# vrettasm/VGPA

Measured on AMD Instinct MI355X. Metric: fwd+bwd sweeps/sec (free-energy+grad eval), Lorenz96 D=40 N=1000, higher is better.
Workload: dtype f64; 1 GPU; Lorenz96 D=40, RK4, Np=1001 (BASELINE configs[2]); batch_per_gpu=512, kernels=mfma

## Files before the change

### vgpa_amd/csrc/energy.hip

```cpp
#include "vgpa_internal.h"
#include "energy_small.h"
#include "chol_wave.h"

namespace vgpa {
namespace {

constexpr int NT = 256;

__global__ void __launch_bounds__(NT) k_energy_1d(EnergyArgs a) {
  const int t = blockIdx.x * NT + threadIdx.x;
  const int prob = blockIdx.y;
  if (t >= a.Np) return;
  const size_t o = (size_t)prob * a.Np + t;
  const double la = a.A[(size_t)prob * a.strideA + t], ob = a.b[(size_t)prob * a.strideB + t], m = a.m[o], s = a.S[o];
  Energy1d r;
  const double th = a.theta_v ? a.theta_v[(size_t)prob * kMaxTheta] : a.theta[0];
  const double sg = a.sigma1_v ? a.sigma1_v[prob] : a.sigma1;
  if (a.model == VGPA_MODEL_OU) energy_1d<VGPA_MODEL_OU>(th, sg, la, ob, m, s, r);
  else energy_1d<VGPA_MODEL_DW>(th, sg, la, ob, m, s, r);
  if (a.hyp_only) { a.hyp[o] = r.hyp; return; }
  a.e_t[o] = r.e_t;
  a.Ef[o] = r.ef;
  if (a.Edf) a.Edf[o] = r.edf;
  a.dEm[o] = r.dm;
  a.dEs[o] = r.ds;
  if (a.hyp) a.hyp[o] = r.hyp;
}

__global__ void __launch_bounds__(64) k_energy_l63(EnergyArgs a) {
  const int t = blockIdx.x * 64 + threadIdx.x;
  const int prob = blockIdx.y;
  if (t >= a.Np) return;
  const size_t o = (size_t)prob * a.Np + t;
  const double* At = a.A + (size_t)prob * a.strideA + (size_t)t * 9;
  const double* bt = a.b + (size_t)prob * a.strideB + (size_t)t * 3;
  const double* mt = a.m + o * 3;
  const double* St = a.S + o * 9;
  double Av[9], bv[3], mv[3], Sv[9], isg[3];
  const double* th = a.theta_v ? a.theta_v + (size_t)prob * kMaxTheta : a.theta;
  const double* isgp = a.isg + (size_t)prob * a.isg_stride;
#pragma unroll
  for (int e = 0; e < 9; e++) { Av[e] = At[e]; Sv[e] = St[e]; }
#pragma unroll
  for (int i = 0; i < 3; i++) { bv[i] = bt[i]; mv[i] = mt[i]; isg[i] = isgp[i]; }
  EnergyL63 r;
  if (a.hyp) energy_l63<true>(th, isg, Av, bv, mv, Sv, r); else energy_l63<false>(th, isg, Av, bv, mv, Sv, r);
  if (a.hyp_only) {
    double* hp = a.hyp + o * 6;
#pragma unroll
    for (int i = 0; i < 6; i++) hp[i] = r.hyp[i];
    return;
  }
  a.e_t[o] = r.e_t;
  double* dm = a.dEm + o * 3;
  dm[0] = r.dm[0]; dm[1] = r.dm[1]; dm[2] = r.dm[2];
  double* ds = a.dEs + o * 9;
  ds[0] = r.ds[0]; ds[1] = r.ds[1]; ds[2] = r.ds[2];
  ds[3] = r.ds[1]; ds[4] = r.ds[3]; ds[5] = r.ds[4];
  ds[6] = r.ds[2]; ds[7] = r.ds[4]; ds[8] = r.ds[5];
  double* ef = a.Ef + o * 3;
// ... 73 lines not shown
      if (!any) continue;
      const double af = pa[kk * 4 * LD + 4 * I];
#pragma unroll
      for (int q = 0; q < g::NQ; q++)
        if (kk >= 4 * q && !(TRI == 1 && 4 * q + 3 < I) && !(TRI == 2 && 4 * q > I)) acc[q * NB + I] = __builtin_amdgcn_mfma_f64_4x4x4f64(af, bq[q], acc[q * NB + I], 0, 0, 0);
    }
    if (g::NLEFT > 0 && kk >= 4 * g::NQ) {
#pragma unroll
      for (int v = 0; v < g::NLEFT; v++) {
        if (MODE == 1 && kk < v * g::G) continue;
        if (TRI == 2 && v * g::G + g::G - 1 < 4 * g::NQ) continue;
        int ib = v * g::G + ileft;
        ib = ib < NB ? ib : NB - 1;
        const double af = pa[kk * 4 * LD + 4 * ib];
        acc[NB * g::NQ + v] = __builtin_amdgcn_mfma_f64_4x4x4f64(af, bl, acc[NB * g::NQ + v], 0, 0, 0);
      }
    }
  }
}

template <int NB>
__device__ __forceinline__ void wave_gemm_elem(int u, int& row, int& col, bool& ok) {
  using g = WaveGemmGeo<NB>;
  const int l = threadIdx.x & 63, r4 = l >> 4, c4 = l & 3, b = (l >> 2) & 3;
  constexpr int rem = g::REM ? g::REM : 1;
  int Ib, Jb;
  if (u < NB * g::NQ) {
    const int q = u / NB;
    Ib = u - q * NB; Jb = 4 * q + b; ok = true;
  } else {
    const int v = u - NB * g::NQ;
    Ib = v * g::G + b / rem; Jb = 4 * g::NQ + b % rem;
    ok = (b < g::G * g::REM) && (Ib < NB);
  }
  row = 4 * Ib + r4; col = 4 * Jb + c4;
}

struct L96Lds {
  double *Lm, *Gm, *mv, *bv, *am, *sg, *vv, *dl, *qq, *rd;
};

__host__ __device__ inline int l96_dp(int D) { return 4 * ((D + 3) / 4); }
__host__ __device__ inline int l96_ld(int D) { return l96_dp(D) + 1; }
__host__ __device__ inline size_t l96_lds_doubles(int D) {
  return (size_t)2 * l96_dp(D) * l96_ld(D) + 7 * (size_t)l96_dp(D) + (2 * D + 1) + 8 + 4 * (size_t)l96_dp(D);
}

template <int NB>
__global__ void __launch_bounds__(64) k_energy_l96(EnergyArgs a) {
  extern __shared__ __attribute__((aligned(16))) double smem[];
  const int D = a.D, M = 2 * D + 1;
  constexpr int Dp = 4 * NB, LD = Dp + 1;
  const int l = threadIdx.x;
  const long long wid = blockIdx.x;
  const int prob = (int)(wid / a.Np), t = (int)(wid - (long long)prob * a.Np);
  const size_t o = (size_t)prob * a.Np + t;
  L96Lds S;
  S.Lm = smem; S.Gm = S.Lm + Dp * LD; S.mv = S.Gm + Dp * LD; S.bv = S.mv + Dp; S.am = S.bv + Dp; S.sg = S.am + Dp;
  S.dl = S.sg + Dp; S.qq = S.dl + Dp; S.rd = S.qq + Dp; S.vv = S.rd + Dp;
  const double* At = a.A + (size_t)prob * a.strideA + (size_t)t * D * D;
  const double* St = a.S + o * D * D;
  const double theta = a.theta_v ? lds_const(a.theta_v, prob * kMaxTheta) : a.theta[0];
  const double kappa = 1.05 * D, c = D + kappa;
  const bool act = l < D;
  const bool pad = l < Dp;
  const int li = pad ? l : Dp - 1;

  for (int e = l; e < Dp * LD; e += 64) { S.Lm[e] = 0.0; S.Gm[e] = 0.0; }
  if (pad) { S.mv[l] = 0.0; S.bv[l] = 0.0; S.sg[l] = 0.0; S.am[l] = 0.0; S.dl[l] = 0.0; S.qq[l] = 0.0; S.rd[l] = 1.0; }
  wave_sync();
  {
    constexpr int EPL = (Dp * Dp + 63) / 64;
    const int DD = D * D;
    const unsigned magic = ((1u << 20) + (unsigned)D - 1u) / (unsigned)D;
#pragma unroll
    for (int q0 = 0; q0 < EPL; q0 += 9) {
      double sv[9], av[9];
#pragma unroll
      for (int u = 0; u < 9; u++) {
        const int e = l + 64 * (q0 + u);
        const bool in = (q0 + u < EPL) && (e < DD);
        sv[u] = in ? St[e] : 0.0;
        av[u] = in ? At[e] : 0.0;
      }
#pragma unroll
      for (int u = 0; u < 9; u++) {
        const int e = l + 64 * (q0 + u);
        if ((q0 + u < EPL) && (e < DD)) {
          const int r = (int)(((unsigned)e * magic) >> 20), cc = e - r * D;
          S.Lm[r * LD + cc] = c * sv[u];
          S.Gm[cc * LD + r] = av[u];
        }
      }
    }
  }
  if (l >= D && pad) S.Lm[l * LD + l] = 1.0;
  if (act) { S.mv[l] = a.m[o * D + l]; S.bv[l] = a.b[(size_t)prob * a.strideB + (size_t)t * D + l]; S.sg[l] = a.isg[(size_t)prob * a.isg_stride + l]; }
  wave_sync();

  const int r4 = l >> 4, c4 = l & 3, b = (l >> 2) & 3;
  bool bad = false;
  double myrd = 1.0;
  const double* lrow_b = S.Lm + (4 * b + c4) * LD + r4;
  double* lout_b = S.Lm + (4 * b + r4) * LD + c4;
#pragma unroll
  for (int p = 0; p < NB; p++) {
    const int j0 = 4 * p;
    if (p > 0) {
      const double* brow = S.Lm + (j0 + c4) * LD + r4;
#pragma unroll
      for (int u = 0; p + 4 * u < NB; u++) {
        const bool full = p + 4 * u + 3 < NB;
        const bool rowok = full || (p + 4 * u + b < NB);
        const double* arow = full ? lrow_b + 4 * (p + 4 * u) * LD
                                  : S.Lm + (4 * (rowok ? p + 4 * u + b : NB - 1) + c4) * LD + r4;
        double uacc = 0.0;
#pragma unroll
        for (int kk = 0; kk < p; kk++) uacc = __builtin_amdgcn_mfma_f64_4x4x4f64(arow[4 * kk], brow[4 * kk], uacc, 0, 0, 0);
        if (rowok) lout_b[4 * (p + 4 * u) * LD + j0] -= uacc;
      }
      wave_sync();
    }
    chol_panel_pivots<LD>(S.Lm, myrd, j0, l, li, pad);
    wave_sync();
  }
  if (pad) S.rd[l] = myrd;
  wave_sync();
// ... 103 lines not shown
  if (l == 0) a.e_t[o] = e_t;
  wave_sync();

  const double* l4_a = S.Lm + c4 * LD + r4;
  const double* xd_a = xdiag + 4 * c4 + r4;
  const double* xd_d = xdiag + 4 * r4 + c4;
#pragma unroll
  for (int I = 0; I < NB; I++) {
    const double* arow = l4_a + 4 * I * LD;
    const double xd = xd_a[16 * I];
    const double xdd = xd_d[16 * I];
#pragma unroll
    for (int u = 0; 4 * u < NB; u++) {
      const int Jb = 4 * u + b;
      const bool colok = (4 * u + 3 < NB) || (Jb < NB);
      double* xcol = S.Gm + r4 * LD + 4 * (colok ? Jb : NB - 1) + c4;
      double xo = 0.0;
      if (4 * u <= I) {
        double tacc = 0.0;
#pragma unroll
        for (int K = 4 * u; K < I; K++) tacc = __builtin_amdgcn_mfma_f64_4x4x4f64(arow[4 * K], xcol[4 * K * LD], tacc, 0, 0, 0);
        const double prod = __builtin_amdgcn_mfma_f64_4x4x4f64(xd, tacc, 0.0, 0, 0, 0);
        xo = (Jb < I) ? -prod : ((Jb == I) ? xdd : 0.0);
      }
      if (colok) xcol[4 * I * LD] = xo;
    }
    wave_sync();
  }

  {
    double s = 0.0;
    for (int k = 0; k < Dp; k++) s = __builtin_fma(S.Gm[k * LD + li], S.dl[k], s);
    if (act) a.dEm[o * D + l] = 0.5 * c * s;
  }
  double* ds = a.dEs + o * D * D;
  {
    double acc[WaveGemmGeo<NB>::NU];
    wave_gemm<NB, 1>(S.Gm, S.Gm, LD, acc, S.qq);
#pragma unroll
    for (int u = 0; u < WaveGemmGeo<NB>::NU; u++) {
      int row, col; bool ok;
      wave_gemm_elem<NB>(u, row, col, ok);
      if (ok && row < D && col < D && (row <= col || !a.ds_upper)) ds[row * D + col] = 0.5 * c * acc[u];
    }
  }

  if (act) {
    const int i = l, ip1 = wrap(i + 1, D), im1 = wrap(i - 1, D), im2 = wrap(i - 2, D);
    const double cxx = St[ip1 * D + im1] - St[im2 * D + im1];
    a.Ef[o * D + i] = cxx + (S.mv[ip1] - S.mv[im2]) * S.mv[im1] - S.mv[i] + theta;
  }
  if (a.Edf) {
    double* ed = a.Edf + o * D * D;
    for (int e = l; e < D * D; e += 64) {
      const int k = e / D, j = e - k * D;
      const int kp1 = wrap(k + 1, D), km1 = wrap(k - 1, D), km2 = wrap(k - 2, D);
      double v = 0.0;
      if (j == k) v = -1.0;
      if (j == kp1) v = S.mv[km1];
      if (j == km2) v = -S.mv[km1];
      if (j == km1) v = S.mv[kp1] - S.mv[km2];
      ed[e] = v;
    }
  }
}

__host__ __device__ inline bool l96r_compact(int D) { return (D + 3) / 4 == 10; }
__host__ __device__ inline size_t l96r_lds_doubles(int D) {
  const size_t dp = l96_dp(D);
  if (l96r_compact(D)) return dp * l96_ld(D) + 5 * dp;
  return dp * l96_ld(D) + 6 * dp + 9 * dp;
}
template <int R>
__device__ __forceinline__ double row_ror_blocks(double v) {
  typedef int i2_t __attribute__((ext_vector_type(2)));
  i2_t x = __builtin_bit_cast(i2_t, v), y;
  y[0] = __builtin_amdgcn_mov_dpp(x[0], 0x120 + 4 * R, 0xf, 0xf, false);
  y[1] = __builtin_amdgcn_mov_dpp(x[1], 0x120 + 4 * R, 0xf, 0xf, false);
  return __builtin_bit_cast(double, y);
}

struct TriRowTab { unsigned char r[2080]; };
constexpr TriRowTab make_tri_row_tab() {
  TriRowTab t{};
  int e = 0;
  for (int r = 0; r < 64; r++)
    for (int c = 0; c <= r; c++) t.r[e++] = (unsigned char)r;
  return t;
}
__device__ __constant__ TriRowTab kTriRow = make_tri_row_tab();

template <int NB, bool TG = false>
__global__ void __launch_bounds__(64) __attribute__((amdgpu_waves_per_eu(NB <= 10 ? 3 : 2, NB <= 10 ? 3 : 2))) k_energy_l96_r(EnergyArgs a) {
  extern __shared__ __attribute__((aligned(16))) double smem[];
  const int D = a.D, M = 2 * D + 1;
  constexpr int Dp = 4 * NB, LD = Dp + 1, NUU = (NB + 3) / 4;
  const int l = threadIdx.x;
  const long long wid = blockIdx.x;
  const int prob = (int)(wid / a.Np);
  const int t = (int)(wid - (long long)prob * a.Np);
  const size_t o = (size_t)prob * a.Np + t;
  L96Lds S;
  constexpr bool CMP = (NB == 10);
  S.Lm = smem; S.Gm = nullptr; S.mv = S.Lm + Dp * LD; S.bv = S.mv + Dp; S.am = S.bv + Dp; S.sg = nullptr;
  S.dl = S.am + Dp; S.qq = S.dl + Dp; S.rd = CMP ? nullptr : S.qq + Dp; S.vv = CMP ? nullptr : S.rd + Dp;
  double* pv = S.vv;
  double* pw = CMP ? nullptr : pv + 4 * Dp;
  double* gb2 = CMP ? nullptr : pw + 4 * Dp;
  double* xdiag = pv;
  auto cg2 = [&](int j) -> double* { return S.Lm + j * LD + Dp; };
  auto cps = [&](int minus, int j) -> double* { return S.Lm + (4 + 2 * minus + (j >= 20 ? 1 : 0)) * LD + (j >= 20 ? j : 20 + j); };
  auto cxd = [&](int I, int r, int c) -> double* { return S.Lm + ((I < 6 ? 0 : 4) + r) * LD + 4 * (I < 6 ? I + 4 : I - 1) + c; };
  const double* At = a.A + (size_t)prob * a.strideA + (size_t)t * D * D;
  const bool spk = a.s_packed != 0;
  const int PK = tri_off(D);
  const double* St = a.S + o * (spk ? PK : D * D);
  const double theta = a.theta_v ? lds_const(a.theta_v, prob * kMaxTheta) : a.theta[0];
  const double kappa = 1.05 * D, c = D + kappa;
  const bool act = l < D;
  const bool pad = l < Dp;
  const int li = pad ? l : Dp - 1;
  const int r4 = l >> 4, c4 = l & 3, b = (l >> 2) & 3;

  constexpr int NUE = 0;
  double af[NUU][NB];
  const int klim = (D - r4 + 3) >> 2;
  auto load_af = [&](int u) {
    const int row = 16 * u + (l & 15);
    const double* ap = At + row * D + r4;
    const int kl = row < D ? klim : 0;
#pragma unroll
    for (int K = 0; K < NB; K++) af[u][K] = (K < kl) ? ap[4 * K] : 0.0;
  };

  double sxa = 0.0, sxb = 0.0, v_m = 0.0, v_b = 0.0, v_sg = 0.0;
  double nsxa = 0.0, nsxb = 0.0;
  const int f_ip1 = wrap(l + 1, D), f_im1 = wrap(l - 1, D), f_im2 = wrap(l - 2, D);
  if (act) v_sg = a.isg[(size_t)prob * a.isg_stride + l];
  auto load_vectors = [&]() {
    if (act) {
      sxa = St[f_ip1 * D + f_im1];
      sxb = St[f_im2 * D + f_im1];
      v_m = a.m[o * D + l];
      v_b = a.b[(size_t)prob * a.strideB + (size_t)t * D + l];
    }
  };
  constexpr int EPK = (Dp * (Dp + 1) / 2 + 63) / 64;
  double sv[EPK];
  int rr[EPK];
  auto request = [&](int tn) {
    const size_t on = (size_t)prob * a.Np + tn;
    const double* Sn = a.S + on * PK;
#pragma unroll
    for (int q = 0; q < EPK; q++) {
      const int e = l + 64 * q;
      sv[q] = e < PK ? Sn[e] : 0.0;
      rr[q] = kTriRow.r[e < PK ? e : 0];
    }
    if (act) {
      nsxa = Sn[tri_idx(f_ip1, f_im1)];
      nsxb = Sn[tri_idx(f_im2, f_im1)];
      v_m = a.m[on * D + l];
      v_b = a.b[(size_t)prob * a.strideB + (size_t)tn * D + l];
    }
  };
  if (spk) request(t);

  if (spk) {
    if (D != Dp) {
      for (int e = l; e < Dp * LD; e += 64) S.Lm[e] = 0.0;
      wave_sync();
    }
    sxa = nsxa; sxb = nsxb;
#pragma unroll
    for (int q = 0; q < EPK; q++) {
      const int e = l + 64 * q;
      if (e < PK) {
        const int r = rr[q];
        S.Lm[r * LD + (e - tri_off(r))] = c * sv[q];
      }
    }
  } else if (D == Dp) {
    constexpr int RCH = Dp <= 44 ? Dp : 32;
    const double* sp = St + li;
#pragma unroll
    for (int q0 = 0; q0 < Dp; q0 += RCH) {
      double sv[RCH];
#pragma unroll
      for (int u = 0; u < RCH; u++) sv[u] = (q0 + u < Dp) ? sp[(q0 + u) * Dp] : 0.0;
      if (q0 == 0) load_vectors();
      if (pad) {
#pragma unroll
        for (int u = 0; u < RCH; u++)
          if (q0 + u < Dp) S.Lm[(q0 + u) * LD + l] = c * sv[u];
      }
    }
  } else {
    load_vectors();
    for (int e = l; e < Dp * LD; e += 64) S.Lm[e] = 0.0;
    wave_sync();
    constexpr int EPL = (Dp * Dp + 63) / 64;
    constexpr int CH = (NB <= 11) ? EPL : 13;
    const int DD = D * D;
    const unsigned magic = ((1u << 20) + (unsigned)D - 1u) / (unsigned)D;
#pragma unroll
    for (int q0 = 0; q0 < EPL; q0 += CH) {
      double sv[CH];
#pragma unroll
      for (int u = 0; u < CH; u++) {
        const int e = l + 64 * (q0 + u);
        const bool in = (q0 + u < EPL) && (e < DD);
        sv[u] = in ? St[e] : 0.0;
      }
#pragma unroll
      for (int u = 0; u < CH; u++) {
        const int e = l + 64 * (q0 + u);
        if ((q0 + u < EPL) && (e < DD)) {
          const int r = (int)(((unsigned)e * magic) >> 20), cc = e - r * D;
          S.Lm[r * LD + cc] = c * sv[u];
        }
      }
    }
  }
  if (l >= D && pad) S.Lm[l * LD + l] = 1.0;
  if (pad) { S.mv[l] = v_m; S.bv[l] = v_b; S.am[l] = 0.0; }
  wave_sync();

  bool bad = false;
  double myrd = 1.0;
  const double* lrow_b = S.Lm + (4 * b + c4) * LD + r4;
  double* lout_b = S.Lm + (4 * b + r4) * LD + c4;
#pragma unroll
  for (int p = 0; p < NB; p++) {
    const int j0 = 4 * p;
    if (p > 0) {
      const double* brow = S.Lm + (j0 + c4) * LD + r4;
#pragma unroll
      for (int u = 0; p + 4 * u < NB; u++) {
        const bool full = p + 4 * u + 3 < NB;
        const bool rowok = full || (p + 4 * u + b < NB);
        const double* arow = full ? lrow_b + 4 * (p + 4 * u) * LD
                                  : S.Lm + (4 * (rowok ? p + 4 * u + b : NB - 1) + c4) * LD + r4;
        double uacc = 0.0;
#pragma unroll
        for (int kk = 0; kk < p; kk++) uacc = __builtin_amdgcn_mfma_f64_4x4x4f64(arow[4 * kk], brow[4 * kk], uacc, 0, 0, 0);
        if (rowok) lout_b[4 * (p + 4 * u) * LD + j0] -= uacc;
      }
      wave_sync();
    }
    chol_panel_pivots<LD>(S.Lm, myrd, j0, l, li, pad);
    wave_sync();
  }
  if (!CMP && pad) S.rd[l] = myrd;
  wave_sync();
  bad = __any(!(myrd > 0.0 && myrd < __builtin_inf()));
  if (bad) {
    if (l == 0) atomicOr(a.status + prob, 1);
    return;
  }
#pragma unroll
  for (int u = NUE; u < NUU; u++) load_af(u);

  double amr[NUU], gacc[NUU][NB];
#pragma unroll
  for (int u = 0; u < NUU; u++) {
    amr[u] = 0.0;
#pragma unroll
    for (int J = 0; J < NB; J++) gacc[u][J] = 0.0;
  }
#pragma unroll
  for (int pass = 0; pass < (NUE < NUU ? 2 : 1); pass++) {
    const int u0 = pass == 0 ? 0 : NUE, u1 = pass == 0 ? NUE : NUU;
#pragma unroll
    for (int K = 0; K < NB; K++) {
      const double mk = S.mv[4 * K + r4];
#pragma unroll
      for (int u = u0; u < u1; u++) amr[u] = __builtin_amdgcn_mfma_f64_4x4x4f64(af[u][K], mk, amr[u], 0, 0, 0);
      const double* lk = S.Lm + (4 * K + r4) * LD + c4;
#pragma unroll
      for (int J = 0; J <= K; J++) {
        const double lf = lk[4 * J];
#pragma unroll
        for (int u = u0; u < u1; u++) gacc[u][J] = __builtin_amdgcn_mfma_f64_4x4x4f64(af[u][K], lf, gacc[u][J], 0, 0, 0);
      }
    }
  }
#pragma unroll
  for (int u = 0; u < NUU; u++) {
    const int i = 16 * u + 4 * b + r4;
    if (c4 == 0 && i < D) { S.am[i] = amr[u]; if (!TG && a.Am) a.Am[o * D + i] = amr[u]; }
  }
  if constexpr (TG) wave_sync();

  if constexpr (!TG) {
#pragma unroll
  for (int u = 0; u < NUU; u++) {
    if (u == 0 || (16 * u <= Dp - 1 && 16 * u + 15 >= Dp - 4)) {
      const int i = 16 * u + 4 * b + r4;
      if constexpr (CMP) {
        if (i == D - 1) {
#pragma unroll
          for (int J = 0; J < NB; J++) *cg2(4 * J + c4) = gacc[u][J];
        }
      }
      double* gdst = (i == 0) ? S.dl : ((i == 1) ? S.qq : ((i == D - 1 && !CMP) ? gb2 : nullptr));
      if (gdst) {
#pragma unroll
        for (int J = 0; J < NB; J++) gdst[4 * J + c4] = gacc[u][J];
      }
    }
  }
  }
  double tg_edge = 0.0;
  if constexpr (TG) {
    const double w0 = kappa / c, w1 = 1.0 / (2.0 * c);
    auto col_of = [&](int q) { return q == 0 ? 0 : (q <= D ? q - 1 : q - 1 - D); };
    auto sgn_of = [&](int q) { return q == 0 ? 0.0 : (q <= D ? 1.0 : -1.0); };
    auto chi = [&](int q, int i) { return S.mv[i] + sgn_of(q) * S.Lm[i * LD + col_of(q)]; };
    const int jc = act ? l : 0;
    const int pP = 1 + jc, pM = 1 + D + jc;
    const int pPm = pP - 1, pPp = pP + 1;
    const int pMm = pM - 1, pMp = wrap(pM + 1, M);
    const double P0 = chi(pPm, D - 2), P1 = chi(pPm, D - 1), P2 = chi(pP, 0), P3 = chi(pP, 1), P4 = chi(pP, 2);
    const double N0 = chi(pMm, D - 2), N1 = chi(pMm, D - 1), N2 = chi(pM, 0), N3 = chi(pM, 1), N4 = chi(pM, 2);
    const double Q0 = chi(pP, D - 3), Q1 = chi(pP, D - 2), Q2 = chi(pP, D - 1), Q3 = chi(pPp, 0);
    const double R0 = chi(pM, D - 3), R1 = chi(pM, D - 2), R2 = chi(pM, D - 1), R3 = chi(pMp, 0);
    double bsum = 0.0;
    {
      const double lin = S.am[0] - S.bv[0];
      bsum += lane_value(v_sg, 0) * ((((P3 - P0) * P1 - P2 + theta) + lin) + (((N3 - N0) * N1 - N2 + theta) + lin));
    }
    {
      const double lin = S.am[1] - S.bv[1];
      bsum += lane_value(v_sg, 1) * ((((P4 - P1) * P2 - P3 + theta) + lin) + (((N4 - N1) * N2 - N3 + theta) + lin));
    }
    {
      const double lin = S.am[D - 1] - S.bv[D - 1];
      bsum += lane_value(v_sg, D - 1) * ((((Q3 - Q0) * Q1 - Q2 + theta) + lin) + (((R3 - R0) * R1 - R2 + theta) + lin));
    }
    double part = 0.0;
    if (act) {
      const int i = l;
      const double xm2 = (i >= 2) ? S.mv[i - 2] : chi(M - 1, D - 2 + i);
      const double xm1 = (i >= 1) ? S.mv[i - 1] : chi(M - 1, D - 1);
      const double x1 = (i + 1 < D) ? S.mv[i + 1] : chi(1, 0);
      const double r0 = ((x1 - xm2) * xm1 - S.mv[i] + theta) + S.am[i] - S.bv[i];
      part += w1 * bsum + w0 * (v_sg * r0);
    }
    tg_edge = part;
  }
  double vp[NB], vm[NB];
  double tgi = 0.0;
#pragma unroll
  for (int J = 0; J < NB; J++) { vp[J] = 0.0; vm[J] = 0.0; }
  {
#pragma clang fp contract(fast)
#pragma unroll
  for (int u = 0; u < NUU; u++) {
    const int i = 16 * u + 4 * b + r4;
    const bool ok = (i >= 2) && (i <= D - 2);
    const int ir = ok ? i : 2;
    const double mm2 = S.mv[ir - 2], mm1 = S.mv[ir - 1], m0 = S.mv[ir], m1 = S.mv[ir + 1];
    const double sgr = __shfl(v_sg, ir, 64);
    const double bvi = S.bv[ir], sgi = ok ? sgr : 0.0, ami = amr[u];
    const double dm = m1 - mm2;
    const double base = dm * mm1 - m0 + theta + ami - bvi;
    const double* lp = S.Lm + (ir - 2) * LD + c4;
#pragma unroll
    for (int J = 0; J < NB; J++) {
      const double e2 = lp[4 * J], e1 = lp[LD + 4 * J], e0 = lp[2 * LD + 4 * J], ep = lp[3 * LD + 4 * J];
      const double gi = gacc[u][J];
      const double dl = ep - e2;
      const double ev = base + dl * e1;
      const double od = dm * e1 + (dl * mm1 + (gi - e0));
      vp[J] = vp[J] + sgi * (ev * ev + od * od);
      vm[J] = vm[J] + sgi * (ev * od);
      if constexpr (TG) tgi = tgi + ((4 * J + c4 < D) ? sgi : 0.0) * ev;
      if (J == NB / 2 - 1 || J == NB - 1) __builtin_amdgcn_sched_barrier(0);
    }
  }
  }
  if constexpr (TG) {
    const double part = wave_sum(tg_edge + 2.0 * (1.0 / (2.0 * c)) * tgi);
    if (l == 0) a.tg[o] = part;
    return;
  }
  {
    double rp[NB], rm[NB];
#pragma unroll
    for (int J = 0; J < NB; J++) {
      rp[J] = __builtin_amdgcn_mfma_f64_4x4x4f64(1.0, vp[J], 0.0, 0, 0, 0);
      rm[J] = __builtin_amdgcn_mfma_f64_4x4x4f64(1.0, vm[J], 0.0, 0, 0, 0);
    }
    if constexpr (CMP) {
#pragma unroll
      for (int J = 0; J < NB; J++) {
        const double p1 = rp[J] + row_ror_blocks<1>(rp[J]), m1 = rm[J] + row_ror_blocks<1>(rm[J]);
        rp[J] = p1 + row_ror_blocks<2>(p1);
        rm[J] = m1 + row_ror_blocks<2>(m1);
      }
      wave_sync();
      if (r4 == 0 && b == 0) {
#pragma unroll
        for (int J = 0; J < NB; J++) {
          *cps(0, 4 * J + c4) = rp[J];
          *cps(1, 4 * J + c4) = rm[J];
        }
      }
    } else
    if (r4 == 0) {
#pragma unroll
      for (int J = 0; J < NB; J++) {
        pv[b * Dp + 4 * J + c4] = rp[J];
        pw[b * Dp + 4 * J + c4] = rm[J];
      }
    }
  }
  wave_sync();

  double vplus = 0.0, vminus = 0.0, v0 = 0.0;
  {
    auto col_of = [&](int q) { return q == 0 ? 0 : (q <= D ? q - 1 : q - 1 - D); };
    auto sgn_of = [&](int q) { return q == 0 ? 0.0 : (q <= D ? 1.0 : -1.0); };
    auto chi = [&](int q, int i) { return S.mv[i] + sgn_of(q) * S.Lm[i * LD + col_of(q)]; };
    const int jc = act ? l : 0;
    {
      double s1, s2;
      if constexpr (CMP) { s1 = *cps(0, jc); s2 = *cps(1, jc); }
      else {
        s1 = (pv[jc] + pv[Dp + jc]) + (pv[2 * Dp + jc] + pv[3 * Dp + jc]);
        s2 = (pw[jc] + pw[Dp + jc]) + (pw[2 * Dp + jc] + pw[3 * Dp + jc]);
      }
      vplus = s1 + 2.0 * s2;
      vminus = s1 - 2.0 * s2;
    }
    const int pP = 1 + jc, pM = 1 + D + jc;
    const int pPm = pP - 1, pPp = pP + 1;
    const int pMm = pM - 1, pMp = wrap(pM + 1, M);
    {
      const double P0 = chi(pPm, D - 2), P1 = chi(pPm, D - 1), P2 = chi(pP, 0), P3 = chi(pP, 1), P4 = chi(pP, 2);
      const double N0 = chi(pMm, D - 2), N1 = chi(pMm, D - 1), N2 = chi(pM, 0), N3 = chi(pM, 1), N4 = chi(pM, 2);
      const double Q0 = chi(pP, D - 3), Q1 = chi(pP, D - 2), Q2 = chi(pP, D - 1), Q3 = chi(pPp, 0);
      const double R0 = chi(pM, D - 3), R1 = chi(pM, D - 2), R2 = chi(pM, D - 1), R3 = chi(pMp, 0);
      const double g0 = S.dl[jc], g1 = S.qq[jc], g2 = CMP ? *cg2(jc) : gb2[jc];
      {
        const double ami = S.am[0], bvi = S.bv[0], sgi = lane_value(v_sg, 0);
        const double ra = ((P3 - P0) * P1 - P2 + theta) + (ami + g0) - bvi;
        const double rb = ((N3 - N0) * N1 - N2 + theta) + (ami - g0) - bvi;
        vplus = __builtin_fma(sgi, ra * ra, vplus);
        vminus = __builtin_fma(sgi, rb * rb, vminus);
      }
      {
        const double ami = S.am[1], bvi = S.bv[1], sgi = lane_value(v_sg, 1);
        const double ra = ((P4 - P1) * P2 - P3 + theta) + (ami + g1) - bvi;
        const double rb = ((N4 - N1) * N2 - N3 + theta) + (ami - g1) - bvi;
        vplus = __builtin_fma(sgi, ra * ra, vplus);
        vminus = __builtin_fma(sgi, rb * rb, vminus);
      }
      {
        const double ami = S.am[D - 1], bvi = S.bv[D - 1], sgi = lane_value(v_sg, D - 1);
        const double ra = ((Q3 - Q0) * Q1 - Q2 + theta) + (ami + g2) - bvi;
        const double rb = ((R3 - R0) * R1 - R2 + theta) + (ami - g2) - bvi;
        vplus = __builtin_fma(sgi, ra * ra, vplus);
        vminus = __builtin_fma(sgi, rb * rb, vminus);
      }
    }
    if (act) {
      const int i = l;
      const double xm2 = (i >= 2) ? S.mv[i - 2] : chi(M - 1, D - 2 + i);
      const double xm1 = (i >= 1) ? S.mv[i - 1] : chi(M - 1, D - 1);
      const double x1 = (i + 1 < D) ? S.mv[i + 1] : chi(1, 0);
      const double r0 = ((x1 - xm2) * xm1 - S.mv[i] + theta) + S.am[i] - S.bv[i];
      v0 = v_sg * (r0 * r0);
    }
    v0 = wave_sum(v0);
  }
  const double w0 = kappa / c, w1 = 1.0 / (2.0 * c);
  const double e_part = act ? (vplus + vminus) : 0.0;
  const double e_t = 0.5 * (w0 * v0 + w1 * wave_sum(e_part));
  wave_sync();
  if (pad) {
    S.dl[l] = act ? w1 * (vplus - vminus) : 0.0;
    S.qq[l] = act ? 0.5 * c * (w1 * (vplus + vminus)) - e_t : 0.0;
  }
  if (l == 0) a.e_t[o] = e_t;
  const int l4 = l < NB ? 4 * l : 0;
  const double rd0 = CMP ? __shfl(myrd, l4, 64) : 0.0, rd1 = CMP ? __shfl(myrd, l4 + 1, 64) : 0.0;
  const double rd2 = CMP ? __shfl(myrd, l4 + 2, 64) : 0.0, rd3 = CMP ? __shfl(myrd, l4 + 3, 64) : 0.0;
  if (l < NB) {
    const double* tb = S.Lm + (4 * l) * LD + 4 * l;
    const double x00 = CMP ? rd0 : S.rd[4 * l], x11 = CMP ? rd1 : S.rd[4 * l + 1], x22 = CMP ? rd2 : S.rd[4 * l + 2], x33 = CMP ? rd3 : S.rd[4 * l + 3];
    const double t10 = tb[LD], t20 = tb[2 * LD], t21 = tb[2 * LD + 1], t30 = tb[3 * LD], t31 = tb[3 * LD + 1], t32 = tb[3 * LD + 2];
    const double x10 = -(t10 * x00) * x11;
    const double x21 = -(t21 * x11) * x22;
    const double x32 = -(t32 * x22) * x33;
    const double x20 = -(t20 * x00 + t21 * x10) * x22;
    const double x31 = -(t31 * x11 + t32 * x21) * x33;
    const double x30 = -(t30 * x00 + t31 * x10 + t32 * x20) * x33;
    if constexpr (CMP) {
      double* x0 = cxd(l, 0, 0);
      x0[0] = x00; x0[1] = 0.0; x0[2] = 0.0; x0[3] = 0.0;
      x0[LD] = x10; x0[LD + 1] = x11; x0[LD + 2] = 0.0; x0[LD + 3] = 0.0;
      x0[2 * LD] = x20; x0[2 * LD + 1] = x21; x0[2 * LD + 2] = x22; x0[2 * LD + 3] = 0.0;
      x0[3 * LD] = x30; x0[3 * LD + 1] = x31; x0[3 * LD + 2] = x32; x0[3 * LD + 3] = x33;
    } else {
    double* xo = xdiag + 16 * l;
    xo[0] = x00; xo[1] = 0.0; xo[2] = 0.0; xo[3] = 0.0;
    xo[4] = x10; xo[5] = x11; xo[6] = 0.0; xo[7] = 0.0;
    xo[8] = x20; xo[9] = x21; xo[10] = x22; xo[11] = 0.0;
    xo[12] = x30; xo[13] = x31; xo[14] = x32; xo[15] = x33;
    }
  }
  wave_sync();

  const double* l4_a = S.Lm + c4 * LD + r4;
  const double* xd_a = xdiag + 4 * c4 + r4;
  const double* xd_d = xdiag + 4 * r4 + c4;
#pragma unroll
  for (int I = 0; I < NB; I++) {
    const double* arow = l4_a + 4 * I * LD;
    const double xd = CMP ? *cxd(I, c4, r4) : xd_a[16 * I];
    const double xdd = CMP ? *cxd(I, r4, c4) : xd_d[16 * I];
    double xo[NUU];
#pragma unroll
    for (int u = 0; u < NUU; u++) {
      const int Jb = 4 * u + b;
      const bool colok = (4 * u + 3 < NB) || (Jb < NB);
      const double* xcol = S.Lm + r4 * LD + 4 * (colok ? Jb : NB - 1) + c4;
      xo[u] = 0.0;
      if (4 * u <= I) {
        double tacc = 0.0;
#pragma unroll
        for (int K = 4 * u; K < I; K++) tacc = __builtin_amdgcn_mfma_f64_4x4x4f64(arow[4 * K], xcol[4 * K * LD], tacc, 0, 0, 0);
        const double prod = __builtin_amdgcn_mfma_f64_4x4x4f64(xd, tacc, 0.0, 0, 0, 0);
        xo[u] = (Jb < I) ? -prod : ((Jb == I) ? xdd : 0.0);
      }
    }
#pragma unroll
    for (int u = 0; u < NUU; u++) {
      const int Jb = 4 * u + b;
      const bool colok = (4 * u + 3 < NB) || (Jb < NB);
      if (colok && (!CMP || Jb <= I)) S.Lm[(4 * I + r4) * LD + 4 * Jb + c4] = xo[u];
    }
    wave_sync();
  }

  {
    double s = 0.0;
    if constexpr (CMP) {
      const bool z0 = li < 4, z1 = li < 8;
#pragma unroll
      for (int k = 0; k < 8; k++) s = __builtin_fma((k < 4 ? z0 : z1) ? S.Lm[k * LD + li] : 0.0, S.dl[k], s);
      for (int k = 8; k < Dp; k++) s = __builtin_fma(S.Lm[k * LD + li], S.dl[k], s);
    } else
    for (int k = 0; k < Dp; k++) s = __builtin_fma(S.Lm[k * LD + li], S.dl[k], s);
    if (act) a.dEm[o * D + l] = 0.5 * c * s;
  }
  double* ds = a.dEs + o * D * D;
  {
    double acc[WaveGemmGeo<NB>::NU];
    if (a.ds_packed) {
      using gg = WaveGemmGeo<NB>;
      double* dsp = a.dEs + o * PK;
      wave_gemm<NB, 1, 2>(S.Lm, S.Lm, LD, acc, S.qq);
#pragma unroll
      for (int u = 0; u < gg::NU; u++) {
        if (u < NB * gg::NQ && 4 * (u / NB) > u % NB) continue;
        if (u >= NB * gg::NQ && (u - NB * gg::NQ) * gg::G + gg::G - 1 < 4 * gg::NQ) continue;
        int row, col; bool ok;
        wave_gemm_elem<NB>(u, row, col, ok);
        if (ok && row < D && col <= row) dsp[tri_off(row) + col] = 0.5 * c * acc[u];
      }
    } else if (a.ds_upper) {
      wave_gemm<NB, 1, 1>(S.Lm, S.Lm, LD, acc, S.qq);
#pragma unroll
      for (int u = 0; u < WaveGemmGeo<NB>::NU; u++) {
        if (u < NB * WaveGemmGeo<NB>::NQ && 4 * (u / NB) + 3 < u % NB) continue;
        int row, col; bool ok;
        wave_gemm_elem<NB>(u, row, col, ok);
        if (ok && row < D && col < D && row <= col) ds[row * D + col] = 0.5 * c * acc[u];
      }
    } else {
      wave_gemm<NB, 1>(S.Lm, S.Lm, LD, acc, S.qq);
#pragma unroll
      for (int u = 0; u < WaveGemmGeo<NB>::NU; u++) {
        int row, col; bool ok;
        wave_gemm_elem<NB>(u, row, col, ok);
        if (ok && row < D && col < D) ds[row * D + col] = 0.5 * c * acc[u];
      }
    }
  }

  if (act) {
    const int i = l, ip1 = wrap(i + 1, D), im1 = wrap(i - 1, D), im2 = wrap(i - 2, D);
    const double cxx = sxa - sxb;
    a.Ef[o * D + i] = cxx + (S.mv[ip1] - S.mv[im2]) * S.mv[im1] - S.mv[i] + theta;
  }
  if (a.Edf) {
    double* ed = a.Edf + o * D * D;
    for (int e = l; e < D * D; e += 64) {
      const int k = e / D, j = e - k * D;
      const int kp1 = wrap(k + 1, D), km1 = wrap(k - 1, D), km2 = wrap(k - 2, D);
      double v = 0.0;
      if (j == k) v = -1.0;
      if (j == kp1) v = S.mv[km1];
      if (j == km2) v = -S.mv[km1];
      if (j == km1) v = S.mv[kp1] - S.mv[km2];
      ed[e] = v;
    }
  }
}

__global__ void __launch_bounds__(NT) k_edf_dense(EnergyArgs a) {
  const int D = a.D;
  const int t = blockIdx.x, prob = blockIdx.y;
  const size_t o = (size_t)prob * a.Np + t;
  const double* mv = a.m + o * D;
  double* ed = a.Edf + o * D * D;
  const double* th = a.theta_v ? a.theta_v + (size_t)prob * kMaxTheta : a.theta;
  for (int e = threadIdx.x; e < D * D; e += NT) {
    const int k = e / D, j = e - k * D;
    double v = 0.0;
    if (a.model == VGPA_MODEL_L96) {
      const int kp1 = wrap(k + 1, D), km1 = wrap(k - 1, D), km2 = wrap(k - 2, D);
      if (j == k) v = -1.0;
      if (j == kp1) v = mv[km1];
      if (j == km2) v = -mv[km1];
      if (j == km1) v = mv[kp1] - mv[km2];
    } else if (a.model == VGPA_MODEL_L63) {
      const double vS = th[0], vR = th[1], vB = th[2];
      const double tab[9] = {-vS, vS, 0.0, vR - mv[2], -1.0, -mv[0], mv[1], mv[0], -vB};
      v = tab[e];
    } else if (a.model == VGPA_MODEL_OU) {
      v = -th[0];
    } else {
      v = 4.0 * (th[0] - 3.0 * (mv[0] * mv[0] + a.S[o]));
    }
    ed[e] = v;
  }
}

}
}

namespace vgpa {

hipError_t launch_energy(const EnergyArgs& a, hipStream_t st) {
  if (a.model == VGPA_MODEL_OU || a.model == VGPA_MODEL_DW) {
    dim3 grid((a.Np + NT - 1) / NT, a.batch);
    hipLaunchKernelGGL(k_energy_1d, grid, dim3(NT), 0, st, a);
  } else if (a.model == VGPA_MODEL_L63) {
    dim3 grid((a.Np + 63) / 64, a.batch);
    hipLaunchKernelGGL(k_energy_l63, grid, dim3(64), 0, st, a);
  } else if (a.model == VGPA_MODEL_L96) {
    if (a.D < 4 || a.D > kMaxSmallD) return hipErrorInvalidValue;
    const bool one_matrix = (a.hyp == nullptr);
    if (a.tg && !one_matrix) return hipErrorInvalidValue;
    size_t lds = (one_matrix ? l96r_lds_doubles(a.D) : l96_lds_doubles(a.D)) * sizeof(double);
    const long long nwaves = (long long)a.Np * a.batch;
    if (nwaves > 0x7fffffffLL) return hipErrorInvalidValue;
#define VGPA_L96_CASE(NBV)                                                                                          \
  case NBV:                                                                                                         \
    if (lds > 48 * 1024)                                                                                            \
      (void)hipFuncSetAttribute(one_matrix ? (const void*)k_energy_l96_r<NBV> : (const void*)k_energy_l96<NBV>,       \
                                hipFuncAttributeMaxDynamicSharedMemorySize, (int)lds);                                \
    if (a.tg) {                                                                                                     \
      if (lds > 48 * 1024)                                                                                          \
        (void)hipFuncSetAttribute((const void*)k_energy_l96_r<NBV, true>, hipFuncAttributeMaxDynamicSharedMemorySize, (int)lds); \
      hipLaunchKernelGGL((k_energy_l96_r<NBV, true>), dim3((unsigned)nwaves), dim3(64), lds, st, a);                  \
    } else                                                                                                          \
    if (one_matrix) hipLaunchKernelGGL(k_energy_l96_r<NBV>, dim3((unsigned)nwaves), dim3(64), lds, st, a);          \
    else hipLaunchKernelGGL(k_energy_l96<NBV>, dim3((unsigned)nwaves), dim3(64), lds, st, a);                        \
    break;
    switch ((a.D + 3) / 4) {
      VGPA_L96_CASE(1) VGPA_L96_CASE(2) VGPA_L96_CASE(3) VGPA_L96_CASE(4) VGPA_L96_CASE(5) VGPA_L96_CASE(6)
      VGPA_L96_CASE(7) VGPA_L96_CASE(8) VGPA_L96_CASE(9) VGPA_L96_CASE(10) VGPA_L96_CASE(11) VGPA_L96_CASE(12)
      VGPA_L96_CASE(13) VGPA_L96_CASE(14) VGPA_L96_CASE(15) VGPA_L96_CASE(16)
      default: return hipErrorInvalidValue;
    }
#undef VGPA_L96_CASE
  } else {
    return hipErrorInvalidValue;
  }
  return hipGetLastError();
}

hipError_t launch_edf(const EnergyArgs& a, hipStream_t st) {
  dim3 grid(a.Np, a.batch);
  hipLaunchKernelGGL(k_edf_dense, grid, dim3(NT), 0, st, a);
  return hipGetLastError();
}

}
```

### vgpa_amd/csrc/vgpa_internal.h

```cpp
#pragma once
#include <hip/hip_runtime.h>
#include <stdint.h>
#include <string>
#include <vector>

#include "../../include/vgpa_hip.h"

namespace vgpa {

#ifdef __HIPCC__
__device__ __forceinline__ int ldu(const int32_t* p, int i) {
  typedef const int32_t __attribute__((address_space(4))) * cptr;
  return ((cptr)p)[i];
}
__device__ __forceinline__ double lds_const(const double* p, int i) {
  typedef const double __attribute__((address_space(4))) * cptr;
  return ((cptr)p)[i];
}
#endif

#ifdef __HIPCC__
__host__ __device__ __forceinline__ int tri_off(int r) { return r * (r + 1) / 2; }
__device__ __forceinline__ int tri_row(int e) {
  int i = (int)((__builtin_sqrtf(8.0f * (float)e + 1.0f) - 1.0f) * 0.5f);
// ... 44 lines not shown
  size_t m0_stride, S0_stride;
  int obs_idx_stride;
  size_t Sigma_stride;
  const double* q_scale_v;
  size_t js_const_stride;
};

struct LaneSweepArgs {
  OdeArgs o;
  int model;
  int want_grad;
  double theta[kMaxTheta];
  double sigma1;
  double isg[4];
  double isig[16];
  double e0, pre, div;
  const double* eobs;
  double* esde;
  double* f;
  double* g;
  const double* e0v;
  const double* theta_v;
  const double* sigma1_v;
  const double* isig_v;
};

struct EnergyArgs {
  int model, D, Np, batch;
  double dt;
  double theta[kMaxTheta];
  double sigma1;
  const double* isg;
  size_t strideA, strideB;
  const double* A;
  const double* b;
  const double* m;
  const double* S;
  double* e_t;
  double* Ef;
  double* Edf;
  double* dEm;
  double* dEs;
  int s_packed;
  int ds_upper;
  int ds_packed;
  double* hyp;
  double* Am;
  int32_t* status;
  const double* theta_v;
  const double* sigma1_v;
  size_t isg_stride;
  double* tg;
  int hyp_only;
};

struct ThetaLaneArgs {
  int model, D, Np, batch, bpad;
  double dt;
  size_t stride_x;
  const double* A;
  const double* b;
  const double* msT;
  double theta[kMaxTheta];
  const double* theta_v;
  double* out;
};

struct ObsArgs {
  int D, Np, batch, n_obs, single;
  const int64_t* obs_t;
  const double* obs_y;
  const double* Q;
  const double* K;
  const double* rinv_diag;
  double obs_const;
  const double* m;
  const double* S;
  double* jm_sparse;
  double* eobs;
  int s_packed;
  int diag;
  double* part;
  size_t obs_t_stride, obs_y_stride;
  size_t Q_stride, K_stride, rinv_stride;
  const double* obs_const_v;
  const int32_t* n_obs_v;
  size_t js_const_stride;
};

struct GradArgs {
  int model, D, Np, batch, sigma_diag;
  int scalar_product;
  double dt;
  double theta[kMaxTheta];
  const double* isig;
  size_t strideA, strideB;
  const double* A; const double* b;
  const double* m; const double* S;
  const double* lam; const double* psi;
  int s_packed;
  int psi_is_q;
  const double* Ef;
  const double* Am;
  const double* Edf;
  double* g;
  const double* theta_v;
// ... 162 lines not shown
```

Baseline: 22160 sweeps/s.

## Use buffer loads/stores with OOB clamping and a 2D grid in L96 energy kernel

Replaces guarded global loads and stores in the L96 energy kernel with AMD raw buffer load/store intrinsics. Out-of-range lanes are given a large offset so the hardware bounds check drops them instead of branching. The launch grid changes from a flat wave index divided by Np to a (t, prob, z) grid, which removes the 64-bit division. The host now precomputes the D magic divisor and passes it in the args. The aim is to cut address arithmetic, divisions and divergent predication in the memory-bound parts. The risk is correctness at the edges, since it relies on buffer OOB semantics and on the padded tri-row table.

```diff
diff --git a/vgpa_amd/csrc/energy.hip b/vgpa_amd/csrc/energy.hip
--- a/vgpa_amd/csrc/energy.hip
+++ b/vgpa_amd/csrc/energy.hip
@@ -6,6 +6,7 @@
 namespace {
 
 constexpr int NT = 256;
+constexpr int kL96ProbsPerZ = 32768;
 
 __global__ void __launch_bounds__(NT) k_energy_1d(EnergyArgs a) {
   const int t = blockIdx.x * NT + threadIdx.x;
@@ -185,8 +186,8 @@
   const int D = a.D, M = 2 * D + 1;
   constexpr int Dp = 4 * NB, LD = Dp + 1;
   const int l = threadIdx.x;
-  const long long wid = blockIdx.x;
-  const int prob = (int)(wid / a.Np), t = (int)(wid - (long long)prob * a.Np);
+  const int prob = (int)(blockIdx.z * kL96ProbsPerZ + blockIdx.y), t = (int)blockIdx.x;
+  if (prob >= a.batch) return;
   const size_t o = (size_t)prob * a.Np + t;
   L96Lds S;
   S.Lm = smem; S.Gm = S.Lm + Dp * LD; S.mv = S.Gm + Dp * LD; S.bv = S.mv + Dp; S.am = S.bv + Dp; S.sg = S.am + Dp;
@@ -205,7 +206,7 @@
   {
     constexpr int EPL = (Dp * Dp + 63) / 64;
     const int DD = D * D;
-    const unsigned magic = ((1u << 20) + (unsigned)D - 1u) / (unsigned)D;
+    const unsigned magic = a.d_magic;
 #pragma unroll
     for (int q0 = 0; q0 < EPL; q0 += 9) {
       double sv[9], av[9];
@@ -415,8 +416,9 @@
   }
   if (a.Edf) {
     double* ed = a.Edf + o * D * D;
+    const unsigned magic = a.d_magic;
     for (int e = l; e < D * D; e += 64) {
-      const int k = e / D, j = e - k * D;
+      const int k = (int)(((unsigned)e * magic) >> 20), j = e - k * D;
       const int kp1 = wrap(k + 1, D), km1 = wrap(k - 1, D), km2 = wrap(k - 2, D);
       double v = 0.0;
       if (j == k) v = -1.0;
@@ -443,15 +445,28 @@
   return __builtin_bit_cast(double, y);
 }
 
-struct TriRowTab { unsigned char r[2080]; };
+struct TriRowTab { unsigned char r[2112]; };
 constexpr TriRowTab make_tri_row_tab() {
   TriRowTab t{};
   int e = 0;
   for (int r = 0; r < 64; r++)
     for (int c = 0; c <= r; c++) t.r[e++] = (unsigned char)r;
+  for (; e < 2112; e++) t.r[e] = 64;
   return t;
 }
 __device__ __constant__ TriRowTab kTriRow = make_tri_row_tab();
+
+typedef unsigned int u2v_t __attribute__((ext_vector_type(2)));
+constexpr int kBeyond = 0x7ff00000;
+__device__ __forceinline__ __amdgpu_buffer_rsrc_t buf_of(const double* p, int doubles) {
+  return __builtin_amdgcn_make_buffer_rsrc(const_cast<double*>(p), 0, p ? doubles * (int)sizeof(double) : 0, 0x00020000);
+}
+__device__ __forceinline__ double buf_load(__amdgpu_buffer_rsrc_t r, int voff) {
+  return __builtin_bit_cast(double, __builtin_amdgcn_raw_buffer_load_b64(r, voff, 0, 0));
+}
+__device__ __forceinline__ void buf_store(__amdgpu_buffer_rsrc_t r, int voff, double v) {
+  __builtin_amdgcn_raw_buffer_store_b64(__builtin_bit_cast(u2v_t, v), r, voff, 0, 0);
+}
 
 template <int NB, bool TG = false>
 __global__ void __launch_bounds__(64) __attribute__((amdgpu_waves_per_eu(NB <= 10 ? 3 : 2, NB <= 10 ? 3 : 2))) k_energy_l96_r(EnergyArgs a) {
@@ -459,9 +474,8 @@
   const int D = a.D, M = 2 * D + 1;
   constexpr int Dp = 4 * NB, LD = Dp + 1, NUU = (NB + 3) / 4;
   const int l = threadIdx.x;
-  const long long wid = blockIdx.x;
-  const int prob = (int)(wid / a.Np);
-  const int t = (int)(wid - (long long)prob * a.Np);
+  const int prob = (int)(blockIdx.z * kL96ProbsPerZ + blockIdx.y), t = (int)blockIdx.x;
+  if (prob >= a.batch) return;
   const size_t o = (size_t)prob * a.Np + t;
   L96Lds S;
   constexpr bool CMP = (NB == 10);
@@ -487,45 +501,41 @@
 
   constexpr int NUE = 0;
   double af[NUU][NB];
-  const int klim = (D - r4 + 3) >> 2;
   auto load_af = [&](int u) {
-    const int row = 16 * u + (l & 15);
-    const double* ap = At + row * D + r4;
-    const int kl = row < D ? klim : 0;
-#pragma unroll
-    for (int K = 0; K < NB; K++) af[u][K] = (K < kl) ? ap[4 * K] : 0.0;
+    const __amdgpu_buffer_rsrc_t rA = buf_of(At, D * D);
+    const int base = 8 * (((l & 15) + 16 * u) * D + r4);
+    const int last = (4 * (NB - 1) + r4 < D) ? base : kBeyond;
+#pragma unroll
+    for (int K = 0; K < NB; K++) af[u][K] = buf_load(rA, (K == NB - 1 ? last : base) + 32 * K);
   };
 
   double sxa = 0.0, sxb = 0.0, v_m = 0.0, v_b = 0.0, v_sg = 0.0;
   double nsxa = 0.0, nsxb = 0.0;
   const int f_ip1 = wrap(l + 1, D), f_im1 = wrap(l - 1, D), f_im2 = wrap(l - 2, D);
-  if (act) v_sg = a.isg[(size_t)prob * a.isg_stride + l];
+  const __amdgpu_buffer_rsrc_t rS = buf_of(St, spk ? PK : D * D);
+  v_sg = buf_load(buf_of(a.isg + (size_t)prob * a.isg_stride, D), 8 * l);
   auto load_vectors = [&]() {
-    if (act) {
-      sxa = St[f_ip1 * D + f_im1];
-      sxb = St[f_im2 * D + f_im1];
-      v_m = a.m[o * D + l];
-      v_b = a.b[(size_t)prob * a.strideB + (size_t)t * D + l];
-    }
+    sxa = buf_load(rS, act ? 8 * (f_ip1 * D + f_im1) : kBeyond);
+    sxb = buf_load(rS, act ? 8 * (f_im2 * D + f_im1) : kBeyond);
+    v_m = buf_load(buf_of(a.m + o * D, D), 8 * l);
+    v_b = buf_load(buf_of(a.b + (size_t)prob * a.strideB + (size_t)t * D, D), 8 * l);
   };
   constexpr int EPK = (Dp * (Dp + 1) / 2 + 63) / 64;
   double sv[EPK];
   int rr[EPK];
   auto request = [&](int tn) {
     const size_t on = (size_t)prob * a.Np + tn;
-    const double* Sn = a.S + on * PK;
-#pragma unroll
-    for (int q = 0; q < EPK; q++) {
-      const int e = l + 64 * q;
-      sv[q] = e < PK ? Sn[e] : 0.0;
-      rr[q] = kTriRow.r[e < PK ? e : 0];
-    }
-    if (act) {
-      nsxa = Sn[tri_idx(f_ip1, f_im1)];
-      nsxb = Sn[tri_idx(f_im2, f_im1)];
-      v_m = a.m[on * D + l];
-      v_b = a.b[(size_t)prob * a.strideB + (size_t)tn * D + l];
-    }
+    const __amdgpu_buffer_rsrc_t rSn = buf_of(a.S + on * PK, PK);
+    const unsigned char* tr = kTriRow.r + l;
+    asm volatile("" : "+v"(tr));
+#pragma unroll
+    for (int q = 0; q < EPK; q++) sv[q] = buf_load(rSn, 8 * l + 512 * q);
+#pragma unroll
+    for (int q = 0; q < EPK; q++) rr[q] = tr[64 * q];
+    nsxa = buf_load(rSn, act ? 8 * tri_idx(f_ip1, f_im1) : kBeyond);
+    nsxb = buf_load(rSn, act ? 8 * tri_idx(f_im2, f_im1) : kBeyond);
+    v_m = buf_load(buf_of(a.m + on * D, D), 8 * l);
+    v_b = buf_load(buf_of(a.b + (size_t)prob * a.strideB + (size_t)tn * D, D), 8 * l);
   };
   if (spk) request(t);
 
@@ -535,22 +545,23 @@
       wave_sync();
     }
     sxa = nsxa; sxb = nsxb;
+    constexpr int TP = Dp * (Dp + 1) / 2;
 #pragma unroll
     for (int q = 0; q < EPK; q++) {
       const int e = l + 64 * q;
-      if (e < PK) {
-        const int r = rr[q];
-        S.Lm[r * LD + (e - tri_off(r))] = c * sv[q];
-      }
+      const int r = rr[q];
+      double* dst = S.Lm + (r * LD + (e - tri_off(r)));
+      if (64 * q + 63 < TP) *dst = c * sv[q];
+      else if (e < TP) *dst = c * sv[q];
     }
   } else if (D == Dp) {
     constexpr int RCH = Dp <= 44 ? Dp : 32;
-    const double* sp = St + li;
+    const int sp = pad ? 8 * l : kBeyond;
 #pragma unroll
     for (int q0 = 0; q0 < Dp; q0 += RCH) {
       double sv[RCH];
 #pragma unroll
-      for (int u = 0; u < RCH; u++) sv[u] = (q0 + u < Dp) ? sp[(q0 + u) * Dp] : 0.0;
+      for (int u = 0; u < RCH; u++) sv[u] = (q0 + u < Dp) ? buf_load(rS, sp + 8 * (q0 + u) * Dp) : 0.0;
       if (q0 == 0) load_vectors();
       if (pad) {
 #pragma unroll
@@ -564,23 +575,20 @@
     wave_sync();
     constexpr int EPL = (Dp * Dp + 63) / 64;
     constexpr int CH = (NB <= 11) ? EPL : 13;
-    const int DD = D * D;
-    const unsigned magic = ((1u << 20) + (unsigned)D - 1u) / (unsigned)D;
+    const unsigned magic = a.d_magic;
 #pragma unroll
     for (int q0 = 0; q0 < EPL; q0 += CH) {
       double sv[CH];
 #pragma unroll
+      for (int u = 0; u < CH; u++) sv[u] = (q0 + u < EPL) ? buf_load(rS, 8 * l + 512 * (q0 + u)) : 0.0;
+#pragma unroll
       for (int u = 0; u < CH; u++) {
         const int e = l + 64 * (q0 + u);
-        const bool in = (q0 + u < EPL) && (e < DD);
-        sv[u] = in ? St[e] : 0.0;
-      }
-#pragma unroll
-      for (int u = 0; u < CH; u++) {
-        const int e = l + 64 * (q0 + u);
-        if ((q0 + u < EPL) && (e < DD)) {
+        if (q0 + u < EPL) {
           const int r = (int)(((unsigned)e * magic) >> 20), cc = e - r * D;
-          S.Lm[r * LD + cc] = c * sv[u];
+          double* dst = S.Lm + (r * LD + cc);
+          if (64 * (q0 + u) + 63 < (Dp - 3) * Dp) *dst = c * sv[u];
+          else if (e < Dp * D) *dst = c * sv[u];
         }
       }
     }
@@ -651,7 +659,8 @@
 #pragma unroll
   for (int u = 0; u < NUU; u++) {
     const int i = 16 * u + 4 * b + r4;
-    if (c4 == 0 && i < D) { S.am[i] = amr[u]; if (!TG && a.Am) a.Am[o * D + i] = amr[u]; }
+    if (c4 == 0 && i < D) S.am[i] = amr[u];
+    if constexpr (!TG) buf_store(buf_of(a.Am ? a.Am + o * D : nullptr, D), (c4 == 0 ? 8 * (4 * b + r4) : kBeyond) + 128 * u, amr[u]);
   }
   if constexpr (TG) wave_sync();
 
@@ -745,7 +754,7 @@
   }
   if constexpr (TG) {
     const double part = wave_sum(tg_edge + 2.0 * (1.0 / (2.0 * c)) * tgi);
-    if (l == 0) a.tg[o] = part;
+    buf_store(buf_of(a.tg + o, 1), 8 * l, part);
     return;
   }
   {
@@ -846,7 +855,7 @@
     S.dl[l] = act ? w1 * (vplus - vminus) : 0.0;
     S.qq[l] = act ? 0.5 * c * (w1 * (vplus + vminus)) - e_t : 0.0;
   }
-  if (l == 0) a.e_t[o] = e_t;
+  buf_store(buf_of(a.e_t + o, 1), 8 * l, e_t);
   const int l4 = l < NB ? 4 * l : 0;
   const double rd0 = CMP ? __shfl(myrd, l4, 64) : 0.0, rd1 = CMP ? __shfl(myrd, l4 + 1, 64) : 0.0;
   const double rd2 = CMP ? __shfl(myrd, l4 + 2, 64) : 0.0, rd3 = CMP ? __shfl(myrd, l4 + 3, 64) : 0.0;
@@ -917,59 +926,82 @@
       for (int k = 8; k < Dp; k++) s = __builtin_fma(S.Lm[k * LD + li], S.dl[k], s);
     } else
     for (int k = 0; k < Dp; k++) s = __builtin_fma(S.Lm[k * LD + li], S.dl[k], s);
-    if (act) a.dEm[o * D + l] = 0.5 * c * s;
-  }
-  double* ds = a.dEs + o * D * D;
+    buf_store(buf_of(a.dEm + o * D, D), 8 * l, 0.5 * c * s);
+  }
   {
-    double acc[WaveGemmGeo<NB>::NU];
+    using gg = WaveGemmGeo<NB>;
+    constexpr int rem = gg::REM ? gg::REM : 1;
+    const bool okL = b < gg::G * gg::REM;
+    const int rlF = r4, clF = 4 * b + c4, rlL = 4 * (b / rem) + r4, clL = 4 * (b % rem) + c4;
+    constexpr int clmaxF = 15, clmaxL = 4 * (rem - 1) + 3, rlmaxF = 3, rlmaxL = 4 * (gg::G > 0 ? gg::G - 1 : 0) + 3;
+    auto unit = [&](int u, bool& left, int& R0, int& C0) {
+      left = u >= NB * gg::NQ;
+      if (!left) { const int q = u / NB; R0 = 4 * (u - q * NB); C0 = 16 * q; }
+      else { R0 = 4 * (u - NB * gg::NQ) * gg::G; C0 = 16 * gg::NQ; }
+    };
+    double acc[gg::NU];
     if (a.ds_packed) {
-      using gg = WaveGemmGeo<NB>;
-      double* dsp = a.dEs + o * PK;
+      const __amdgpu_buffer_rsrc_t rD = buf_of(a.dEs + o * PK, PK);
+      const int pkF = 8 * (tri_off(rlF) + clF), pkL = okL ? 8 * (tri_off(rlL) + clL) : kBeyond;
+      const int dF = clF - rlF, dL = clL - rlL;
       wave_gemm<NB, 1, 2>(S.Lm, S.Lm, LD, acc, S.qq);
 #pragma unroll
       for (int u = 0; u < gg::NU; u++) {
         if (u < NB * gg::NQ && 4 * (u / NB) > u % NB) continue;
         if (u >= NB * gg::NQ && (u - NB * gg::NQ) * gg::G + gg::G - 1 < 4 * gg::NQ) continue;
-        int row, col; bool ok;
-        wave_gemm_elem<NB>(u, row, col, ok);
-        if (ok && row < D && col <= row) dsp[tri_off(row) + col] = 0.5 * c * acc[u];
+        bool left; int R0, C0;
+        unit(u, left, R0, C0);
+        int off = (left ? pkL : pkF) + (8 * R0) * (left ? rlL : rlF) + 8 * (tri_off(R0) + C0);
+        if (R0 - C0 < (left ? clmaxL : clmaxF)) off = ((left ? dL : dF) <= R0 - C0) ? off : kBeyond;
+        buf_store(rD, off, 0.5 * c * acc[u]);
       }
     } else if (a.ds_upper) {
+      const __amdgpu_buffer_rsrc_t rD = buf_of(a.dEs + o * D * D, D * D);
+      const int whF = 8 * (rlF * D + clF), whL = okL ? 8 * (rlL * D + clL) : kBeyond;
+      const int dF = clF - rlF, dL = clL - rlL;
       wave_gemm<NB, 1, 1>(S.Lm, S.Lm, LD, acc, S.qq);
 #pragma unroll
-      for (int u = 0; u < WaveGemmGeo<NB>::NU; u++) {
-        if (u < NB * WaveGemmGeo<NB>::NQ && 4 * (u / NB) + 3 < u % NB) continue;
-        int row, col; bool ok;
-        wave_gemm_elem<NB>(u, row, col, ok);
-        if (ok && row < D && col < D && row <= col) ds[row * D + col] = 0.5 * c * acc[u];
+      for (int u = 0; u < gg::NU; u++) {
+        if (u < NB * gg::NQ && 4 * (u / NB) + 3 < u % NB) continue;
+        bool left; int R0, C0;
+        unit(u, left, R0, C0);
+        int off = (left ? whL : whF) + 8 * (R0 * D + C0);
+        if (R0 - C0 > -(left ? rlmaxL : rlmaxF)) off = ((left ? dL : dF) >= R0 - C0) ? off : kBeyond;
+        if (C0 + (left ? clmaxL : clmaxF) >= Dp - 3) off = ((left ? clL : clF) < D - C0) ? off : kBeyond;
+        buf_store(rD, off, 0.5 * c * acc[u]);
       }
     } else {
+      const __amdgpu_buffer_rsrc_t rD = buf_of(a.dEs + o * D * D, D * D);
+      const int whF = 8 * (rlF * D + clF), whL = okL ? 8 * (rlL * D + clL) : kBeyond;
       wave_gemm<NB, 1>(S.Lm, S.Lm, LD, acc, S.qq);
 #pragma unroll
-      for (int u = 0; u < WaveGemmGeo<NB>::NU; u++) {
-        int row, col; bool ok;
-        wave_gemm_elem<NB>(u, row, col, ok);
-        if (ok && row < D && col < D) ds[row * D + col] = 0.5 * c * acc[u];
-      }
-    }
-  }
-
-  if (act) {
-    const int i = l, ip1 = wrap(i + 1, D), im1 = wrap(i - 1, D), im2 = wrap(i - 2, D);
+      for (int u = 0; u < gg::NU; u++) {
+        bool left; int R0, C0;
+        unit(u, left, R0, C0);
+        int off = (left ? whL : whF) + 8 * (R0 * D + C0);
+        if (C0 + (left ? clmaxL : clmaxF) >= Dp - 3) off = ((left ? clL : clF) < D - C0) ? off : kBeyond;
+        buf_store(rD, off, 0.5 * c * acc[u]);
+      }
+    }
+  }
+
+  {
+    const int i = act ? l : 0, ip1 = wrap(i + 1, D), im1 = wrap(i - 1, D), im2 = wrap(i - 2, D);
     const double cxx = sxa - sxb;
-    a.Ef[o * D + i] = cxx + (S.mv[ip1] - S.mv[im2]) * S.mv[im1] - S.mv[i] + theta;
+    buf_store(buf_of(a.Ef + o * D, D), 8 * l, cxx + (S.mv[ip1] - S.mv[im2]) * S.mv[im1] - S.mv[i] + theta);
   }
   if (a.Edf) {
-    double* ed = a.Edf + o * D * D;
+    const __amdgpu_buffer_rsrc_t rE = buf_of(a.Edf + o * D * D, D * D);
+    const unsigned magic = a.d_magic;
     for (int e = l; e < D * D; e += 64) {
-      const int k = e / D, j = e - k * D;
+      const int k = (int)(((unsigned)e * magic) >> 20), j = e - k * D;
       const int kp1 = wrap(k + 1, D), km1 = wrap(k - 1, D), km2 = wrap(k - 2, D);
       double v = 0.0;
       if (j == k) v = -1.0;
       if (j == kp1) v = S.mv[km1];
       if (j == km2) v = -S.mv[km1];
       if (j == km1) v = S.mv[kp1] - S.mv[km2];
-      ed[e] = v;
+      buf_store(rE, 8 * e, v);
     }
   }
 }
@@ -1008,7 +1040,9 @@
 
 namespace vgpa {
 
-hipError_t launch_energy(const EnergyArgs& a, hipStream_t st) {
+hipError_t launch_energy(const EnergyArgs& args, hipStream_t st) {
+  EnergyArgs a = args;
+  a.d_magic = a.D > 0 ? ((1u << 20) + (unsigned)a.D - 1u) / (unsigned)a.D : 0u;
   if (a.model == VGPA_MODEL_OU || a.model == VGPA_MODEL_DW) {
     dim3 grid((a.Np + NT - 1) / NT, a.batch);
     hipLaunchKernelGGL(k_energy_1d, grid, dim3(NT), 0, st, a);
@@ -1022,6 +1056,8 @@
     size_t lds = (one_matrix ? l96r_lds_doubles(a.D) : l96_lds_doubles(a.D)) * sizeof(double);
     const long long nwaves = (long long)a.Np * a.batch;
     if (nwaves > 0x7fffffffLL) return hipErrorInvalidValue;
+    const int per_z = a.batch < kL96ProbsPerZ ? a.batch : kL96ProbsPerZ;
+    const dim3 grid((unsigned)a.Np, (unsigned)per_z, (unsigned)((a.batch + kL96ProbsPerZ - 1) / kL96ProbsPerZ));
 #define VGPA_L96_CASE(NBV)                                                                                          \
   case NBV:                                                                                                         \
     if (lds > 48 * 1024)                                                                                            \
@@ -1030,10 +1066,10 @@
     if (a.tg) {                                                                                                     \
       if (lds > 48 * 1024)                                                                                          \
         (void)hipFuncSetAttribute((const void*)k_energy_l96_r<NBV, true>, hipFuncAttributeMaxDynamicSharedMemorySize, (int)lds); \
-      hipLaunchKernelGGL((k_energy_l96_r<NBV, true>), dim3((unsigned)nwaves), dim3(64), lds, st, a);                  \
+      hipLaunchKernelGGL((k_energy_l96_r<NBV, true>), grid, dim3(64), lds, st, a);                  \
     } else                                                                                                          \
-    if (one_matrix) hipLaunchKernelGGL(k_energy_l96_r<NBV>, dim3((unsigned)nwaves), dim3(64), lds, st, a);          \
-    else hipLaunchKernelGGL(k_energy_l96<NBV>, dim3((unsigned)nwaves), dim3(64), lds, st, a);                        \
+    if (one_matrix) hipLaunchKernelGGL(k_energy_l96_r<NBV>, grid, dim3(64), lds, st, a);          \
+    else hipLaunchKernelGGL(k_energy_l96<NBV>, grid, dim3(64), lds, st, a);                        \
     break;
     switch ((a.D + 3) / 4) {
       VGPA_L96_CASE(1) VGPA_L96_CASE(2) VGPA_L96_CASE(3) VGPA_L96_CASE(4) VGPA_L96_CASE(5) VGPA_L96_CASE(6)
diff --git a/vgpa_amd/csrc/vgpa_internal.h b/vgpa_amd/csrc/vgpa_internal.h
--- a/vgpa_amd/csrc/vgpa_internal.h
+++ b/vgpa_amd/csrc/vgpa_internal.h
@@ -120,6 +120,7 @@
   size_t isg_stride;
   double* tg;
   int hyp_only;
+  unsigned d_magic;
 };
 
 struct ThetaLaneArgs {
```

New measurement: 22340 sweeps/s, median of 6. Within noise of the previous version (+0.8%).
